# thangvubk/PESR

Measured on AMD Instinct MI355X. Metric: HR-patches/sec (x4 SR GAN train step, 48->192), higher is better.
Workload: dtype f32; 1 GPU; full GAN phase (G + D + VGG + RSGAN focal loss), per-GPU batch 16, LR 48x48 -> HR 192x192, 256 ch x 32 blocks; Adam lr 5e-07 instead of the reference's 5e-5 (same work per step; keeps D's loss O(0.1) on white-noise crops, see `lr_note`); global_batch=16, parallelism=dp1

## Files before the change

pesr_amd/csrc/conv3x3_mfma.hip:

```cpp
#include <mutex>
#include "common.h"
#include "launchers.h"
#include "conv_epilogue.h"

__device__ __attribute__((aligned(16))) const float g_zero16[4] = {0.f, 0.f, 0.f, 0.f};

__device__ __forceinline__ void lds_dma16(const float* gsrc, char* lds_wave_base) {
    __builtin_amdgcn_global_load_lds((const __attribute__((address_space(1))) void*)gsrc,
                                     (__attribute__((address_space(3))) void*)lds_wave_base, 16, 0, 0);
}

struct ConvArgs {
    const float* x;
    const float* wp;
    const float* bias;
    const float* skip;
    const float* mask;
    float* y;
    int N, H, W, Cin, Cout, OH, OW;
    int GH, GW;
    int TH, TW, tiles_x, tiles_y, n_tiles;
    int in_oy, in_ox;
    int HT, WT;
    int out_my, out_ay, out_mx, out_ax;
    int ntaps;
    unsigned long long tap_lo;
    unsigned tap_hi;
    float alpha, slope;
    int act;
    int ps;
    int cin_real;
    int cout_store;
    int ksplit;
    int chunks_per_split;
    float* slab;
    size_t slab_bytes;
    int ps_in;
    int bn_row0;
    int bn_mode, bn_cap;
    int dry;
    long bn_rows;
};

__device__ __forceinline__ unsigned tap_code(const ConvArgs& a, int t) {
    return t < 8 ? (unsigned)(a.tap_lo >> (8 * t)) & 0xffu : a.tap_hi;
}

template <int WAVES_M, int WAVES_N, int WM, int WN, int S, int HL, int MODE>
__device__ __forceinline__ void conv3x3_mfma_body(const ConvArgs& a, const int block_id, const int grid_blocks, const unsigned bn_kernarg_off) {
    constexpr int NT = WAVES_M * WAVES_N * 64;
    constexpr int BN = WAVES_N * WN * 16;
    constexpr int WL = (BN * 4 + NT - 1) / NT;
    extern __shared__ __attribute__((aligned(16))) char smem[];

    const int halo_pix = a.HT * a.WT;
    const int halo_bytes = ((halo_pix * 64 + 255) / 256) * 256;
    char* const halo0 = smem;
    char* const halo1 = smem + halo_bytes;
    char* const wb0 = smem + 2 * halo_bytes;

    const int tid = threadIdx.x, lane = tid & 63, wave = tid >> 6;
    const int wave_m = wave / WAVES_N, wave_n = wave % WAVES_N;
    const int r = lane & 15, g = lane >> 4;

    int lb = block_id;
    if ((grid_blocks & 7) == 0) lb = (lb & 7) * (grid_blocks >> 3) + (lb >> 3);
    const int tiles_total = a.n_tiles * a.tiles_x * a.tiles_y * a.N;
    const int ks = lb / tiles_total;
    int bid = lb - ks * tiles_total;
    const int nt = bid % a.n_tiles;  bid /= a.n_tiles;
    const int tx = bid % a.tiles_x;  bid /= a.tiles_x;
    const int ty = bid % a.tiles_y;
    const int img = bid / a.tiles_y;
    const int gy0 = ty * a.TH, gx0 = tx * a.TW;
    const int n0 = nt * BN;
    const int C16T = a.Cin >> 4;
    const int CB = ks * a.chunks_per_split;
    const int C16 = (C16T - CB) < a.chunks_per_split ? (C16T - CB) : a.chunks_per_split;

    int a_off[WM], b_off[WN];
#pragma unroll
    for (int i = 0; i < WM; ++i) {
        const int m = (wave_m * WM + i) * 16 + r;
        const int py = m / a.TW, px = m - py * a.TW;
        a_off[i] = ((py * S) * a.WT + (S == 2 ? px : px * S)) * 64 + g * 16;
    }
    const int WE = (a.WT + 1) >> 1;
#pragma unroll
    for (int j = 0; j < WN; ++j) b_off[j] = ((wave_n * WN + j) * 16 + r) * 64 + g * 16;

    const float* const xi = a.x + (size_t)img * a.H * a.W * a.cin_real;
    int h_src[HL];
#pragma unroll
    for (int k = 0; k < HL; ++k) {
        const int e = tid + k * NT;
        const int hp = e >> 2, q = e & 3;
        int off = -2;
        if (hp < halo_pix) {
            const int hy = hp / a.WT, sc = hp - hy * a.WT;
            const int hx = S == 2 ? (sc < WE ? 2 * sc : 2 * (sc - WE) + 1) : sc;
            const int iy = gy0 * S + a.in_oy + hy, ix = gx0 * S + a.in_ox + hx;
            if (iy >= 0 && iy < a.H && ix >= 0 && ix < a.W)
                off = a.ps_in ? ((2 * iy) * (2 * a.W) + 2 * ix) * (a.Cin >> 2) + q * 4 : (iy * a.W + ix) * a.cin_real + q * 4;
            else
                off = -1;
        }
        h_src[k] = off;
    }
    const float* const wn = a.wp + (size_t)n0 * 16;
    const size_t slab_stride = (size_t)a.Cout * 16;

    f32x4 acc[WM][WN];
#pragma unroll
    for (int i = 0; i < WM; ++i)
#pragma unroll
        for (int j = 0; j < WN; ++j) acc[i][j] = (f32x4){0.f, 0.f, 0.f, 0.f};

    f32x4 hreg[HL], wreg[WL];

    auto load_halo = [&](int c) {
        int coff = (CB + c) * 16;
        if (a.ps_in) coff = pesr_ps_in_chunk_off(coff, a.Cin >> 2, a.W);
        if (a.cin_real == 3) {
#pragma unroll
            for (int k = 0; k < HL; ++k) {
                const bool ok = h_src[k] >= 0 && ((tid + k * NT) & 3) == 0;
                const int o = ok ? h_src[k] : 0;
                const float v0 = xi[o], v1 = xi[o + 1], v2 = xi[o + 2];
                hreg[k] = ok ? (f32x4){v0, v1, v2, 0.f} : (f32x4){0.f, 0.f, 0.f, 0.f};
            }
            return;
        }
#pragma unroll
        for (int k = 0; k < HL; ++k) {
            const int o = h_src[k] < 0 ? 0 : h_src[k];
            f32x4 v = *(const f32x4*)(xi + o + coff);
            hreg[k] = h_src[k] >= 0 ? v : (f32x4){0.f, 0.f, 0.f, 0.f};
        }
    };
    auto store_halo = [&](char* hb) {
#pragma unroll
        for (int k = 0; k < HL; ++k)
            if (h_src[k] != -2) *(f32x4*)(hb + (tid + k * NT) * 16) = hreg[k];
    };
    auto load_w = [&](int c, int tw) {
        const float* src = wn + ((size_t)tw * C16T + CB + c) * slab_stride;
#pragma unroll
        for (int k = 0; k < WL; ++k) {
            const int e = tid + k * NT;
            if (BN * 4 % NT == 0 || e < BN * 4) wreg[k] = *(const f32x4*)(src + e * 4);
        }
    };
    auto store_w = [&](char* wb) {
#pragma unroll
        for (int k = 0; k < WL; ++k) {
            const int e = tid + k * NT;
            if (BN * 4 % NT == 0 || e < BN * 4) *(f32x4*)(wb + e * 16) = wreg[k];
        }
    };

    auto dma_w = [&](int c, int tw, char* wb) {
        const float* src = wn + ((size_t)tw * C16T + CB + c) * slab_stride;
#pragma unroll
        for (int k = 0; k < WL; ++k) {
            const int e = tid + k * NT;
            if (BN * 4 % NT == 0 || e < BN * 4) lds_dma16(src + e * 4, wb + (k * NT + wave * 64) * 16);
        }
    };
    auto dma_halo = [&](int c, char* hb) {
        int coff = (CB + c) * 16;
        if (a.ps_in) coff = pesr_ps_in_chunk_off(coff, a.Cin >> 2, a.W);
#pragma unroll
        for (int k = 0; k < HL; ++k) {
            if (h_src[k] != -2) {
                const float* src = h_src[k] >= 0 ? xi + h_src[k] + coff : g_zero16;
                lds_dma16(src, hb + (k * NT + wave * 64) * 16);
            }
        }
    };

    f32x4 fa0[WM], fb0[WN], fa1[WM], fb1[WN];

#define PESR_READ_FRAGS(FA, FB, C_, T_, WB_)                                                    \
    {                                                                                          \
        const char* const hb_ = ((C_) & 1) ? halo1 : halo0;                                    \
        const unsigned tc_ = tap_code(a, T_);                                                  \
        const int dx_ = (int)((tc_ >> 2) & 3u);                                                \
        const int toff_ = ((int)(tc_ & 3u) * a.WT + (S == 2 ? (dx_ == 1 ? WE : dx_ >> 1) : dx_)) * 64; \
        _Pragma("unroll") for (int i = 0; i < WM; ++i) FA[i] = *(const f32x4*)(hb_ + a_off[i] + toff_); \
        _Pragma("unroll") for (int j = 0; j < WN; ++j) FB[j] = *(const f32x4*)((WB_) + b_off[j]); \
    }
#define PESR_MFMA_BLOCK(FA, FB)                                                                 \
    _Pragma("unroll") for (int kk = 0; kk < 4; ++kk)                                            \
        _Pragma("unroll") for (int i = 0; i < WM; ++i)                                          \
            _Pragma("unroll") for (int j = 0; j < WN; ++j)                                      \
                acc[i][j] = __builtin_amdgcn_mfma_f32_16x16x4f32(FA[i][kk], FB[j][kk], acc[i][j], 0, 0, 0);

    const int nslab = C16 * a.ntaps;
    auto adv = [&](int& c_, int& t_) { if (++t_ == a.ntaps) { t_ = 0; if (++c_ == C16) c_ = 0; } };

    if (MODE == 2) {
        char* const ring = wb0;
        int cd = 0, td = 0, sd = 0;
        auto dma_next = [&]() { dma_w(cd, tap_code(a, td) >> 4, ring + (sd & 3) * (BN * 64)); adv(cd, td); ++sd; };
        dma_halo(0, halo0);
        dma_next(); dma_next(); dma_next();
        __syncthreads();
        int cr = 0, tr = 0, sr = 0;
        PESR_READ_FRAGS(fa0, fb0, cr, tr, ring + (sr & 3) * (BN * 64))  adv(cr, tr); ++sr;
        __syncthreads();
        int c = 0, t = 0;
#pragma unroll 1
        for (int sl = 0; sl < nslab; sl += 2) {
            dma_next(); dma_next();
            {
                int c1 = c, t1 = t; adv(c1, t1);
                const int copen = (t == 0) ? c : ((t1 == 0 && sl + 1 < nslab) ? c1 : -1);
                if (copen >= 0 && copen + 1 < C16 && (t == 0 || c1 != 0)) dma_halo(copen + 1, ((copen + 1) & 1) ? halo1 : halo0);
            }
            PESR_READ_FRAGS(fa1, fb1, cr, tr, ring + (sr & 3) * (BN * 64))  adv(cr, tr); ++sr;
            PESR_MFMA_BLOCK(fa0, fb0)
            adv(c, t);
            if (sl + 1 < nslab) {
                PESR_READ_FRAGS(fa0, fb0, cr, tr, ring + (sr & 3) * (BN * 64))  adv(cr, tr); ++sr;
                PESR_MFMA_BLOCK(fa1, fb1)
                adv(c, t);
            }
            __syncthreads();
        }
    } else {
        auto wslot = [&](int s_) -> char* { return wb0 + (MODE == 0 ? s_ % 3 : (s_ & 1)) * (BN * 64); };
        load_halo(0);
        load_w(0, tap_code(a, 0) >> 4);
        store_halo(halo0);
        store_w(wslot(0));
        if (nslab > 1) {
            int c1 = 0, t1 = 0; adv(c1, t1);
            load_w(c1, tap_code(a, t1) >> 4);
            store_w(wslot(1));
        }
        __syncthreads();
        if (MODE == 1) PESR_READ_FRAGS(fa0, fb0, 0, 0, wslot(0))
        int c = 0, t = 0;
#define PESR_STEP(CA, CB_, NA, NB, SL)                                                          \
        {                                                                                      \
            int c1 = c, t1 = t; adv(c1, t1);                                                   \
            int c2 = c1, t2 = t1; adv(c2, t2);                                                 \
            const bool halo_now = (t == 0) && (c + 1 < C16);                                   \
            load_w(c2, tap_code(a, t2) >> 4);                                                  \
            if (halo_now) load_halo(c + 1);                                                    \
            if (MODE == 1) PESR_READ_FRAGS(NA, NB, c1, t1, wslot((SL) + 1))                    \
            else PESR_READ_FRAGS(CA, CB_, c, t, wslot(SL))                                     \
            PESR_MFMA_BLOCK(CA, CB_)                                                           \
                        \
            __builtin_amdgcn_sched_barrier(0);                                                 \
            store_w(wslot((SL) + 2));        \
            if (halo_now) store_halo((c & 1) ? halo0 : halo1);                                 \
            __syncthreads();                                                                   \
            c = c1; t = t1;                                                                    \
        }
#pragma unroll 1
        for (int sl = 0; sl < nslab; sl += 2) {
            PESR_STEP(fa0, fb0, fa1, fb1, sl)
            if (sl + 1 < nslab) PESR_STEP(fa1, fb1, fa0, fb0, sl + 1)
        }
#undef PESR_STEP
    }
#undef PESR_MFMA_BLOCK
#undef PESR_READ_FRAGS

    const size_t img_out = (size_t)img * a.OH * a.OW;
    if (a.cout_store % 4 == 0) {
        constexpr int MT = WAVES_M * WM * 16;
        constexpr int C4 = BN / 4;
        constexpr int RS = BN * 4 + 16;
        constexpr int EIT = (MT * C4 + NT - 1) / NT;
        char* const ob = smem;
        const BnEpi* const bn = pesr_bn_epi(bn_kernarg_off);
        const int bn_mode = a.ksplit == 1 ? bn->mode : 0;
        const bool bn_on = bn_mode != 0;
        const float bn_slope = bn->slope;
        f32x4 st1 = {0.f, 0.f, 0.f, 0.f}, st2 = {0.f, 0.f, 0.f, 0.f};
        PesrBnCoef4 bnk = pesr_bn_coef4_zero();
        auto out_index = [&](int u, size_t* idx) -> bool {
            const int m = u / C4, c4 = u - m * C4;
            const int co = n0 + c4 * 4;
            const int py = m / a.TW, px = m - py * a.TW;
            const int gy = gy0 + py, gx = gx0 + px;
            if (u >= MT * C4 || gy >= a.GH || gx >= a.GW || co >= a.cout_store) return false;
            const int oy = gy * a.out_my + a.out_ay, ox = gx * a.out_mx + a.out_ax;
            if (a.ps) {
                *idx = pesr_ps_out_index(img, oy, ox, co, a.OH, a.OW, a.Cout);
            } else {
                *idx = (img_out + (size_t)oy * a.OW + ox) * a.cout_store + co;
            }
            return true;
        };
        f32x4 zpre[EIT];
        if (bn_mode == 2) {
            const int cq = n0 + (tid % C4) * 4;
            if (cq < a.cout_store) bnk = pesr_bn_coef4_load(bn, a.cout_store, cq);
        }
#pragma unroll
        for (int i = 0; i < WM; ++i)
#pragma unroll
            for (int jj = 0; jj < 4; ++jj) {
                const int m = (wave_m * WM + i) * 16 + g * 4 + jj;
#pragma unroll
                for (int j = 0; j < WN; ++j)
                    *(float*)(ob + m * RS + ((wave_n * WN + j) * 16 + r) * 4) = acc[i][j][jj];
            }
        __syncthreads();
        const size_t slab_off = (size_t)ks * ((size_t)a.N * a.OH * a.OW * a.cout_store);
        if (bn_mode == 2) {
            {
                const float* const bn_z = bn->z;
#pragma unroll
                for (int k = 0; k < EIT; ++k) {
                    size_t idx;
                    zpre[k] = out_index(tid + k * NT, &idx) ? *(const f32x4*)(bn_z + idx) : (f32x4){0.f, 0.f, 0.f, 0.f};
                }
            }
#pragma unroll
            for (int k = 0; k < EIT; ++k) {
                const int u = tid + k * NT;
                size_t idx;
                if (!out_index(u, &idx)) continue;
                const int m = u / C4, c4 = u - m * C4;
                const f32x4 v = pesr_bn_lrelu_grad4(*(const f32x4*)(ob + m * RS + c4 * 16) * a.alpha, zpre[k], bnk, bn_slope, st1, st2);
                *(f32x4*)(a.y + idx) = v;
            }
        } else {
            for (int u = tid; u < MT * C4; u += NT) {
                size_t idx;
                if (!out_index(u, &idx)) continue;
                const int m = u / C4, c4 = u - m * C4;
                const int co = n0 + c4 * 4;
                f32x4 v = *(const f32x4*)(ob + m * RS + c4 * 16);
                if (a.ksplit > 1) {
                    *(f32x4*)(a.slab + slab_off + idx) = v;
                    continue;
                }
                v = pesr_epi4_at(v, a.bias, co, a.alpha, a.mask, a.skip, idx, a.act, a.slope);
                if (bn_on) { st1 += v; st2 += v * v; }
                *(f32x4*)(a.y + idx) = v;
            }
        }
        if (bn_on) {
            __syncthreads();
            f32x4* const red = (f32x4*)smem;
            red[tid] = st1; red[NT + tid] = st2;
            __syncthreads();
            if (tid < C4 && n0 + tid * 4 < a.cout_store) {
                f64x4 d1 = {0.0, 0.0, 0.0, 0.0}, d2 = {0.0, 0.0, 0.0, 0.0};
                for (int k = 0; k < NT / C4; ++k) {
                    d1 += __builtin_convertvector(red[k * C4 + tid], f64x4);
                    d2 += __builtin_convertvector(red[NT + k * C4 + tid], f64x4);
                }
                const int row = a.bn_row0 + (img * a.tiles_y + ty) * a.tiles_x + tx;
                float* const pr = bn->part + (size_t)row * 2 * a.cout_store + n0 + tid * 4;
                *(f32x4*)pr = __builtin_convertvector(d1, f32x4);
                *(f32x4*)(pr + a.cout_store) = __builtin_convertvector(d2, f32x4);
            }
        }
        return;
    }
    float bias_r[WN];
#pragma unroll
    for (int j = 0; j < WN; ++j) {
        const int co = n0 + (wave_n * WN + j) * 16 + r;
        bias_r[j] = (a.bias && co < a.cout_store) ? a.bias[co] : 0.f;
    }
#pragma unroll
    for (int i = 0; i < WM; ++i) {
#pragma unroll
        for (int jj = 0; jj < 4; ++jj) {
            const int m = (wave_m * WM + i) * 16 + g * 4 + jj;
            const int py = m / a.TW, px = m - py * a.TW;
            const int gy = gy0 + py, gx = gx0 + px;
            if (gy >= a.GH || gx >= a.GW) continue;
            const int oy = gy * a.out_my + a.out_ay, ox = gx * a.out_mx + a.out_ax;
#pragma unroll
            for (int j = 0; j < WN; ++j) {
                const int co = n0 + (wave_n * WN + j) * 16 + r;
                if (co >= a.cout_store) continue;
                size_t idx;
                if (a.ksplit > 1) {
                    idx = (img_out + (size_t)oy * a.OW + ox) * a.cout_store + co;
                    a.slab[(size_t)ks * ((size_t)a.N * a.OH * a.OW * a.cout_store) + idx] = acc[i][j][jj];
                    continue;
                }
                if (a.ps) idx = pesr_ps_out_index(img, oy, ox, co, a.OH, a.OW, a.Cout);
                else idx = (img_out + (size_t)oy * a.OW + ox) * a.cout_store + co;
                a.y[idx] = pesr_epi1_at(acc[i][j][jj] + bias_r[j], nullptr, 0, a.alpha, a.mask, a.skip, idx, a.act, a.slope);
            }
        }
    }
}

template <int WAVES_M, int WAVES_N, int WM, int WN, int S, int HL, int MODE>
__global__ __launch_bounds__(WAVES_M* WAVES_N * 64) void conv3x3_mfma_kernel(const ConvArgs a, const BnEpi bn) {
    (void)bn;
    conv3x3_mfma_body<WAVES_M, WAVES_N, WM, WN, S, HL, MODE>(a, blockIdx.x, gridDim.x, (unsigned)((sizeof(ConvArgs) + 7) & ~(size_t)7));
}

struct ConvArgs4 {
    ConvArgs c[4];
    int tiles[4];
};
template <int WAVES_M, int WAVES_N, int WM, int WN, int HL>
__global__ __launch_bounds__(WAVES_M* WAVES_N * 64) void conv3x3_s2dgrad4_kernel(const ConvArgs4 a4, const BnEpi bn) {
    (void)bn;
    constexpr unsigned BO = (unsigned)((sizeof(ConvArgs4) + 7) & ~(size_t)7);
    const int bx = blockIdx.x;
    switch (blockIdx.y) {
        case 0: if (bx < a4.tiles[0]) conv3x3_mfma_body<WAVES_M, WAVES_N, WM, WN, 1, HL, 2>(a4.c[0], bx, a4.tiles[0], BO); break;
        case 1: if (bx < a4.tiles[1]) conv3x3_mfma_body<WAVES_M, WAVES_N, WM, WN, 1, HL, 1>(a4.c[1], bx, a4.tiles[1], BO); break;
        case 2: if (bx < a4.tiles[2]) conv3x3_mfma_body<WAVES_M, WAVES_N, WM, WN, 1, HL, 1>(a4.c[2], bx, a4.tiles[2], BO); break;
        default: if (bx < a4.tiles[3]) conv3x3_mfma_body<WAVES_M, WAVES_N, WM, WN, 1, HL, 0>(a4.c[3], bx, a4.tiles[3], BO); break;
    }
}

__global__ void conv_splitk_finish_kernel(const float* __restrict__ slab, const float* __restrict__ bias, const float* __restrict__ skip,
                                          const float* __restrict__ mask, float* __restrict__ y, long total, int C, int ksplit,
                                          float alpha, int act, float slope) {
    for (long e = (long)blockIdx.x * blockDim.x + threadIdx.x; e < total; e += (long)gridDim.x * blockDim.x) {
        float v = slab[e];
        for (int k = 1; k < ksplit; ++k) v += slab[(size_t)k * total + e];
        y[e] = pesr_epi1_at(v, bias, bias ? e % C : 0, alpha, mask, skip, e, act, slope);
    }
}
__global__ void conv_splitk_finish4_kernel(const f32x4* __restrict__ slab, const float* __restrict__ bias, const f32x4* __restrict__ skip,
                                           const f32x4* __restrict__ mask, f32x4* __restrict__ y, long total4, int C, int ksplit,
                                           float alpha, int act, float slope) {
    for (long e = (long)blockIdx.x * blockDim.x + threadIdx.x; e < total4; e += (long)gridDim.x * blockDim.x) {
        f32x4 p[8];
#pragma unroll
        for (int k = 0; k < 8; ++k)
            if (k < ksplit) p[k] = slab[(size_t)k * total4 + e];
        f32x4 v = p[0];
#pragma unroll
        for (int k = 1; k < 8; ++k)
            if (k < ksplit) v += p[k];
        y[e] = pesr_epi4_at(v, bias, (e * 4) % C, alpha, (const float*)mask, (const float*)skip, e * 4, act, slope);
    }
}

constexpr int PESR_BN_FINISH_ROWS = 256;
template <int MODE>
__global__ __launch_bounds__(256) void conv_splitk_finish4_bn_kernel(const f32x4* __restrict__ slab, const float* __restrict__ bias, f32x4* __restrict__ y,
                                                                      long total4, int C, int ksplit, float alpha, const BnEpi bn) {
    const int C4 = C >> 2;
    const int c4 = (int)(((long)blockIdx.x * 256 + threadIdx.x) % C4);
    f32x4 st1 = {0.f, 0.f, 0.f, 0.f}, st2 = st1, b4 = st1;
    PesrBnCoef4 bnk = pesr_bn_coef4_zero();
    if (MODE == 2) bnk = pesr_bn_coef4_load(&bn, C, c4 * 4);
    if (bias) b4 = *(const f32x4*)(bias + c4 * 4);
    for (long e = (long)blockIdx.x * 256 + threadIdx.x; e < total4; e += (long)gridDim.x * 256) {
        f32x4 p[8];
#pragma unroll
        for (int k = 0; k < 8; ++k)
            if (k < ksplit) p[k] = slab[(size_t)k * total4 + e];
        f32x4 v = p[0];
#pragma unroll
        for (int k = 1; k < 8; ++k)
            if (k < ksplit) v += p[k];
        v = (v + b4) * alpha;
        if (MODE == 2) {
            v = pesr_bn_lrelu_grad4(v, ((const f32x4*)bn.z)[e], bnk, bn.slope, st1, st2);
        } else {
            st1 += v; st2 += v * v;
        }
        y[e] = v;
    }
    __shared__ f32x4 red[2][256];
    red[0][threadIdx.x] = st1; red[1][threadIdx.x] = st2;
    __syncthreads();
    const int cw = C4 < 256 ? C4 : 256;
    if (threadIdx.x < cw) {
        f64x4 d1 = {0.0, 0.0, 0.0, 0.0}, d2 = {0.0, 0.0, 0.0, 0.0};
        for (int k = threadIdx.x; k < 256; k += cw) {
            d1 += __builtin_convertvector(red[0][k], f64x4);
            d2 += __builtin_convertvector(red[1][k], f64x4);
        }
        float* const pr = bn.part + (size_t)blockIdx.x * 2 * C + c4 * 4;
        *(f32x4*)pr = __builtin_convertvector(d1, f32x4);
        *(f32x4*)(pr + C) = __builtin_convertvector(d2, f32x4);
    }
}

long pesr_conv_splitk_finish_bn_rows(int C, int ksplit) {
    const int C4 = C >> 2;
    if (C % 4 || ksplit > 8 || C4 < 1 || (C4 < 256 ? 256 % C4 : C4 % 256)) return 0;
    return PESR_BN_FINISH_ROWS;
}

int pesr_conv_splitk_finish_bn_launch(const float* slab, const float* bias, float* y, long total, int C, int ksplit, float alpha, const BnEpi& bn,
                                      hipStream_t stream) {
    if (!pesr_conv_splitk_finish_bn_rows(C, ksplit) || !bn.part) return PESR_EINVAL;
    const long total4 = total / 4;
    if (bn.mode == 2)
        hipLaunchKernelGGL(conv_splitk_finish4_bn_kernel<2>, dim3(PESR_BN_FINISH_ROWS), dim3(256), 0, stream, (const f32x4*)slab, bias, (f32x4*)y, total4, C, ksplit,
                           alpha, bn);
    else
        hipLaunchKernelGGL(conv_splitk_finish4_bn_kernel<1>, dim3(PESR_BN_FINISH_ROWS), dim3(256), 0, stream, (const f32x4*)slab, bias, (f32x4*)y, total4, C, ksplit,
                           alpha, bn);
    return pesr_launch_status();
}

int pesr_conv_splitk_finish_launch(const float* slab, const float* bias, const float* skip, const float* mask, float* y, long total,
                                   int C, int ksplit, float alpha, int act, float slope, hipStream_t stream) {
    if (C % 4 == 0 && ksplit <= 8) {
        const long total4 = total / 4;
        const int fgrid = (int)((total4 + 255) / 256 < 4096 ? (total4 + 255) / 256 : 4096);
        hipLaunchKernelGGL(conv_splitk_finish4_kernel, dim3(fgrid), dim3(256), 0, stream, (const f32x4*)slab, bias, (const f32x4*)skip,
                           (const f32x4*)mask, (f32x4*)y, total4, C, ksplit, alpha, act, slope);
        return pesr_launch_status();
    }
    const int fgrid = (int)((total + 255) / 256 < 2048 ? (total + 255) / 256 : 2048);
    hipLaunchKernelGGL(conv_splitk_finish_kernel, dim3(fgrid), dim3(256), 0, stream, slab, bias, skip, mask, y, total, C, ksplit, alpha,
                       act, slope);
    return pesr_launch_status();
}

namespace {

static thread_local BnEpi g_bn_epi;

static void set_tap(ConvArgs& a, int t, int dy, int dx, int w) {
    const unsigned long long code = (unsigned)(dy | (dx << 2) | (w << 4));
    if (t < 8) a.tap_lo |= code << (8 * t); else a.tap_hi = (unsigned)code;
}

struct TileChoice { int TH, TW; };

static bool choose_tile(int MT, int S, int hext, int wext, int GH, int GW, int max_halo_pix, TileChoice* out) {
    long best = -1;
    for (int TW = 1; TW <= MT; ++TW) {
        if (MT % TW) continue;
        const int TH = MT / TW;
        const int HTl = (TH - 1) * S + hext, WTl = (TW - 1) * S + wext;
        if ((long)HTl * WTl > max_halo_pix) continue;
        const long cover = (long)pesr_cdiv(GH, TH) * TH * pesr_cdiv(GW, TW) * TW;
        const long score = cover * 4096 + (long)HTl * WTl;
        if (best < 0 || score < best) { best = score; out->TH = TH; out->TW = TW; }
    }
    return best >= 0;
}

template <int WAVES_M, int WAVES_N, int WM, int WN, int S, int HL>
static int prep_cfg(ConvArgs& a, int hext, int wext, int target_wgs, size_t* lds_out, int* mode_out, long* grid_out) {
    constexpr int NT = WAVES_M * WAVES_N * 64;
    constexpr int MT = WAVES_M * WM * 16;
    constexpr int BN = WAVES_N * WN * 16;
    if (a.Cout % BN) return PESR_EINVAL;
    TileChoice tc;
    const int max_halo = (HL * NT) / 4;
    if (!choose_tile(MT, S, hext, wext, a.GH, a.GW, max_halo, &tc)) return PESR_EINVAL;
    a.TH = tc.TH; a.TW = tc.TW;
    a.HT = (a.TH - 1) * S + hext; a.WT = (a.TW - 1) * S + wext;
    a.tiles_y = pesr_cdiv(a.GH, a.TH); a.tiles_x = pesr_cdiv(a.GW, a.TW);
    a.n_tiles = a.Cout / BN;
    const int halo_bytes = ((a.HT * a.WT * 64 + 255) / 256) * 256;
    const int mode = (a.ntaps >= 4 && a.cin_real != 3) ? 2 : (a.ntaps > 1 ? 1 : 0);
    size_t lds = 2 * (size_t)halo_bytes + (mode == 2 ? 4 : (mode == 0 ? 3 : 2)) * (size_t)BN * 64;
    const size_t lds_acc = (size_t)MT * (BN * 4 + 16);
    if (lds_acc > lds) lds = lds_acc;
    if (lds > 160 * 1024) return PESR_EINVAL;
    const long tiles = (long)a.N * a.tiles_y * a.tiles_x * a.n_tiles;
    const int C16T = a.Cin / 16;
    a.ksplit = 1; a.chunks_per_split = C16T;
    const size_t out_bytes = (size_t)a.N * a.OH * a.OW * a.cout_store * sizeof(float);
    if (a.slab && tiles < (long)target_wgs * 5 / 8 && a.out_my == 1 && a.out_mx == 1 && !a.ps && C16T >= 8) {
        int want = (int)((target_wgs + tiles - 1) / tiles);
        if (want > 8) want = 8;
        if (want > C16T / 4) want = C16T / 4;
        while (want > 1 && (size_t)want * out_bytes > a.slab_bytes) --want;
        if (want > 1) {
            a.chunks_per_split = (C16T + want - 1) / want;
            a.ksplit = (C16T + a.chunks_per_split - 1) / a.chunks_per_split;
        }
    }
    *lds_out = lds; *mode_out = mode; *grid_out = tiles * a.ksplit;
    return PESR_OK;
}

template <int WAVES_M, int WAVES_N, int WM, int WN, int S, int HL>
static int launch_cfg(ConvArgs& a, int hext, int wext, hipStream_t stream, int target_wgs = 256) {
    constexpr int NT = WAVES_M * WAVES_N * 64;
    size_t lds; int mode; long grid;
    const int rc = prep_cfg<WAVES_M, WAVES_N, WM, WN, S, HL>(a, hext, wext, target_wgs, &lds, &mode, &grid);
    if (rc) return rc;
    a.bn_rows = (a.cout_store % 4 == 0 && NT % (WAVES_N * WN * 4) == 0 && !a.ps)
                    ? (a.ksplit == 1 ? (long)a.N * a.tiles_y * a.tiles_x : pesr_conv_splitk_finish_bn_rows(a.cout_store, a.ksplit)) : 0;
    if (a.dry) return PESR_OK;
    if (a.bn_mode && (a.bn_rows == 0 || a.bn_row0 + a.bn_rows != a.bn_cap || !g_bn_epi.part)) return PESR_EINVAL;
    const size_t out_bytes = (size_t)a.N * a.OH * a.OW * a.cout_store * sizeof(float);
    const float* bias = a.bias; const float* skip = a.skip; const float* mask = a.mask;
    BnEpi a_bn = g_bn_epi;
    if (a.ksplit > 1) a_bn.mode = 0;
#define PESR_LAUNCH_MODE(M_)                                                                              \
    {                                                                                                      \
        auto kern = conv3x3_mfma_kernel<WAVES_M, WAVES_N, WM, WN, S, HL, M_>;                              \
        static PesrDeviceOnce attr_once;                                        \
        attr_once([&] {                                                           \
            (void)hipFuncSetAttribute((const void*)kern, hipFuncAttributeMaxDynamicSharedMemorySize, 160 * 1024); \
        });                                                                                                  \
        hipLaunchKernelGGL(kern, dim3((unsigned)grid), dim3(NT), lds, stream, a, a_bn);                    \
    }
    if (mode == 2) PESR_LAUNCH_MODE(2) else if (mode == 1) PESR_LAUNCH_MODE(1) else PESR_LAUNCH_MODE(0)
#undef PESR_LAUNCH_MODE
    if (a.ksplit > 1 && g_bn_epi.mode) {
        if (skip || mask || a.act != PESR_ACT_NONE) return PESR_EINVAL;
        return pesr_conv_splitk_finish_bn_launch((const float*)a.slab, bias, a.y, (long)(out_bytes / sizeof(float)), a.cout_store, a.ksplit, a.alpha,
                                                 g_bn_epi, stream);
    }
    if (a.ksplit > 1)
        return pesr_conv_splitk_finish_launch((const float*)a.slab, bias, skip, mask, a.y, (long)(out_bytes / sizeof(float)), a.cout_store,
                                              a.ksplit, a.alpha, a.act, a.slope, stream);
    return pesr_launch_status();
}

template <int WAVES_M, int WAVES_N, int WM, int WN, int HL>
static int launch_s2dgrad4(ConvArgs4& a4, const int* hext, const int* wext, hipStream_t stream) {
    constexpr int NT = WAVES_M * WAVES_N * 64;
    size_t lds = 0; long gmax = 0;
    long rows = 0;
    const bool rows_ok = a4.c[0].cout_store % 4 == 0 && NT % (WAVES_N * WN * 4) == 0;
    for (int k = 0; k < 4; ++k) {
        a4.tiles[k] = 0;
        a4.c[k].bn_row0 = (int)rows;
        if (a4.c[k].GH <= 0 || a4.c[k].GW <= 0) continue;
        size_t l; int mode; long grid;
        const int rc = prep_cfg<WAVES_M, WAVES_N, WM, WN, 1, HL>(a4.c[k], hext[k], wext[k], 256, &l, &mode, &grid);
        if (rc) return rc;
        if (mode != (k == 0 ? 2 : (k == 3 ? 0 : 1)) || a4.c[k].ksplit != 1) return PESR_EINVAL;
        a4.tiles[k] = (int)grid;
        rows += (long)a4.c[k].N * a4.c[k].tiles_y * a4.c[k].tiles_x;
        if (l > lds) lds = l;
        if (grid > gmax) gmax = grid;
    }
    a4.c[0].bn_rows = rows_ok ? rows : 0;
    if (a4.c[0].dry) return PESR_OK;
    if (a4.c[0].bn_mode && (!rows_ok || rows != a4.c[0].bn_cap || !g_bn_epi.part)) return PESR_EINVAL;
    if (gmax == 0) return PESR_OK;
    auto kern = conv3x3_s2dgrad4_kernel<WAVES_M, WAVES_N, WM, WN, HL>;
    static PesrDeviceOnce attr_once;
    attr_once([&] { (void)hipFuncSetAttribute((const void*)kern, hipFuncAttributeMaxDynamicSharedMemorySize, 160 * 1024); });
    hipLaunchKernelGGL(kern, dim3((unsigned)gmax, 4), dim3(NT), lds, stream, a4, g_bn_epi);
    return pesr_launch_status();
}

template <int S>
static int dispatch(ConvArgs& a, int hext, int wext, hipStream_t stream) {
    const long M = (long)a.N * a.GH * a.GW;
    if (S == 2 && a.ntaps == 9 && a.Cout == 64 && M >= 64 * 512) return launch_cfg<1, 4, 4, 1, S, 5>(a, hext, wext, stream);
    if (a.Cout % 64 == 0 && a.Cout >= 128 && (long)pesr_cdiv(M, 144) * (a.Cout / 64) <= 320)
        return launch_cfg<1, 4, 3, 1, S, (S == 1 ? 2 : 4)>(a, hext, wext, stream, 768);
    if (a.Cout % 256 == 0) {
        const long tiles_big = (M / 144) * (a.Cout / 256);
        if (tiles_big >= 192) return launch_cfg<1, 8, 9, 2, S, (S == 1 ? 2 : 6)>(a, hext, wext, stream);
    }
    if (a.Cout % 128 == 0) {
        const long tiles = (M / 144) * (a.Cout / 128);
        if (tiles >= 192) return launch_cfg<1, 8, 9, 1, S, (S == 1 ? 2 : 6)>(a, hext, wext, stream);
    }
    if (a.Cout % 64 == 0) return launch_cfg<1, 4, 9, 1, S, (S == 1 ? 4 : 11)>(a, hext, wext, stream);
    if (a.Cout == 16 && S == 1) return launch_cfg<4, 1, 4, 1, 1, 6>(a, hext, wext, stream);
    return PESR_EINVAL;
}

}

static void set_bn(ConvArgs& a, PesrBnFuseArgs* f) {
    a.bn_mode = 0; a.dry = 0; a.bn_rows = 0; a.bn_row0 = 0; a.bn_cap = 0;
    g_bn_epi = BnEpi{};
    if (!f) return;
    a.dry = f->dry;
    if (f->dry || !f->mode) return;
    a.bn_mode = f->mode; a.bn_cap = f->rows;
    g_bn_epi.mode = f->mode; g_bn_epi.slope = f->slope; g_bn_epi.part = f->part;
    g_bn_epi.z = f->z; g_bn_epi.mi = f->mean_invstd; g_bn_epi.gamma = f->gamma; g_bn_epi.beta = f->beta;
}

int pesr_conv3x3_launch(const float* x, const float* wp, const float* bias, const float* skip, const float* mask,
                        float* y, int N, int H, int W, int Cin, int Cout, int stride, float alpha, int act,
                        float slope, int ps, int ps_in, int flip, int cin_real, int cout_store, void* ws, size_t ws_bytes,
                        hipStream_t stream, PesrBnFuseArgs* fuse) {
    if (cin_real == 0) cin_real = Cin;
    if (cout_store == 0) cout_store = Cout;
    if ((cin_real != Cin && (cin_real != 3 || Cin != 16 || ps_in)) || (cout_store != Cout && ps)) return PESR_EINVAL;
    if (ps_in && (Cin % 64 || stride != 1)) return PESR_EINVAL;
    if (ps && Cout % 4) return PESR_EINVAL;
    if (Cin % 16 || (stride != 1 && stride != 2) || N <= 0 || H <= 0 || W <= 0) return PESR_EINVAL;
    ConvArgs a{};
    a.x = x; a.wp = wp; a.bias = bias; a.skip = skip; a.mask = mask; a.y = y;
    a.N = N; a.H = H; a.W = W; a.Cin = Cin; a.Cout = Cout;
    a.OH = (H - 1) / stride + 1; a.OW = (W - 1) / stride + 1;
    a.GH = a.OH; a.GW = a.OW;
    a.in_oy = -1; a.in_ox = -1;
    a.out_my = 1; a.out_ay = 0; a.out_mx = 1; a.out_ax = 0;
    a.ntaps = 9;
    for (int t = 0; t < 9; ++t) set_tap(a, t, t / 3, t % 3, flip ? 8 - t : t);
    a.alpha = alpha; a.slope = slope; a.act = act; a.ps = ps; a.ps_in = ps_in;
    a.cin_real = cin_real; a.cout_store = cout_store;
    a.slab = (float*)ws; a.slab_bytes = ws_bytes;
    set_bn(a, fuse);
    if (fuse && fuse->mode == 2 && (mask || skip || bias || act != PESR_ACT_NONE)) return PESR_EINVAL;
    const int rc = stride == 1 ? dispatch<1>(a, 3, 3, stream) : dispatch<2>(a, 3, 3, stream);
    if (fuse) fuse->rows_out = rc ? 0 : a.bn_rows;
    return rc;
}

int pesr_conv3x3_s2_dgrad_launch(const float* dy, const float* wp, const float* mask, float* dx, int N, int H, int W,
                                 int Cout_fwd, int Cin_fwd, float alpha, hipStream_t stream, PesrBnFuseArgs* fuse) {
    if (Cout_fwd % 16) return PESR_EINVAL;
    const int OH = (H - 1) / 2 + 1, OW = (W - 1) / 2 + 1;
    ConvArgs4 a4{};
    int hext[4], wext[4];
    for (int k = 0; k < 4; ++k) {
        const int py = k < 2 ? 1 : 0, px = (k == 0 || k == 2) ? 1 : 0;
        ConvArgs& a = a4.c[k];
        a.x = dy; a.wp = wp; a.bias = nullptr; a.skip = nullptr; a.mask = mask; a.y = dx;
        a.N = N; a.H = OH; a.W = OW; a.Cin = Cout_fwd; a.Cout = Cin_fwd;
        a.OH = H; a.OW = W;
        a.GH = (H - py + 1) / 2; a.GW = (W - px + 1) / 2;
        a.in_oy = 0; a.in_ox = 0;
        a.out_my = 2; a.out_ay = py; a.out_mx = 2; a.out_ax = px;
        int kys[2], dys[2], nky, kxs[2], dxs[2], nkx;
        if (py == 0) { nky = 1; kys[0] = 1; dys[0] = 0; } else { nky = 2; kys[0] = 0; dys[0] = 1; kys[1] = 2; dys[1] = 0; }
        if (px == 0) { nkx = 1; kxs[0] = 1; dxs[0] = 0; } else { nkx = 2; kxs[0] = 0; dxs[0] = 1; kxs[1] = 2; dxs[1] = 0; }
        a.ntaps = 0;
        for (int i = 0; i < nky; ++i)
            for (int j = 0; j < nkx; ++j) {
                set_tap(a, a.ntaps, dys[i], dxs[j], kys[i] * 3 + kxs[j]);
                ++a.ntaps;
            }
        a.alpha = alpha; a.slope = 0.f; a.act = PESR_ACT_NONE; a.ps = 0; a.ps_in = 0;
        a.cin_real = Cout_fwd; a.cout_store = Cin_fwd;
        a.slab = nullptr; a.slab_bytes = 0; a.ksplit = 1;
        set_bn(a, fuse);
        hext[k] = py + 1; wext[k] = px + 1;
    }
    if (fuse && fuse->mode == 2 && mask) return PESR_EINVAL;
    if (fuse) fuse->rows_out = 0;
    const int Cout = Cin_fwd;
    const long M = (long)N * a4.c[0].GH * a4.c[0].GW;
    if (Cout % 64) {
        if (fuse && !fuse->dry && fuse->mode) return PESR_EINVAL;
        if (fuse && fuse->dry) return PESR_OK;
        for (int k = 0; k < 4; ++k) {
            if (a4.c[k].GH <= 0 || a4.c[k].GW <= 0) continue;
            const int rc = dispatch<1>(a4.c[k], hext[k], wext[k], stream);
            if (rc) return rc;
        }
        return PESR_OK;
    }
    int rc;
    if (Cout >= 128 && (long)pesr_cdiv(M, 144) * (Cout / 64) <= 320) rc = launch_s2dgrad4<1, 4, 3, 1, 2>(a4, hext, wext, stream);
    else if (Cout % 256 == 0 && 4 * (M / 144) * (Cout / 256) >= 192) rc = launch_s2dgrad4<1, 8, 9, 2, 2>(a4, hext, wext, stream);
    else if (Cout % 128 == 0 && 4 * (M / 144) * (Cout / 128) >= 192) rc = launch_s2dgrad4<1, 8, 9, 1, 2>(a4, hext, wext, stream);
    else rc = launch_s2dgrad4<1, 4, 9, 1, 4>(a4, hext, wext, stream);
    if (fuse) fuse->rows_out = rc ? 0 : a4.c[0].bn_rows;
    return rc;
}
```

Measured before the change: 304.0 patches/s.

## Add MODE 3 conv path streaming weights from global into registers

Adds a new conv3x3 MFMA kernel mode for single-wave-row, stride-2, 9-tap configurations. Weights are loaded straight from global memory into registers three taps ahead, instead of being DMA'd into an LDS ring, which frees LDS and removes barriers for weight staging. The halo is still double-buffered in LDS through register fetch-and-land, with one barrier per channel chunk. This trades LDS traffic and synchronisation for more VGPR pressure and exposed global-load latency. It is on by default and can be turned off with an environment variable.

```diff
diff --git a/pesr_amd/csrc/conv3x3_mfma.hip b/pesr_amd/csrc/conv3x3_mfma.hip
--- a/pesr_amd/csrc/conv3x3_mfma.hip
+++ b/pesr_amd/csrc/conv3x3_mfma.hip
@@ -199,7 +199,99 @@
     const int nslab = C16 * a.ntaps;
     auto adv = [&](int& c_, int& t_) { if (++t_ == a.ntaps) { t_ = 0; if (++c_ == C16) c_ = 0; } };
 
-    if (MODE == 2) {
+    if (MODE == 3) {
+        static_assert(MODE != 3 || WAVES_M == 1, "MODE 3: the weights are not shared between waves");
+        constexpr int NT3 = 9;
+        const float* wl[WN];
+#pragma unroll
+        for (int j = 0; j < WN; ++j) wl[j] = wn + (b_off[j] >> 2);
+        f32x4 fa[2][WM], fb[3][WN];
+        auto fetch_halo = [&](int c_) {
+            int coff = (CB + c_) * 16;
+            if (a.ps_in) coff = pesr_ps_in_chunk_off(coff, a.Cin >> 2, a.W);
+#pragma unroll
+            for (int k = 0; k < HL; ++k) hreg[k] = *(const f32x4*)(xi + (h_src[k] < 0 ? 0 : h_src[k]) + coff);
+        };
+        auto land_halo = [&](char* hb) {
+#pragma unroll
+            for (int k = 0; k < HL; ++k)
+                if (h_src[k] != -2) *(f32x4*)(hb + (tid + k * NT) * 16) = h_src[k] >= 0 ? hreg[k] : (f32x4){0.f, 0.f, 0.f, 0.f};
+        };
+        auto load_b = [&](f32x4* FB, int c_, int t_) {
+#ifndef PESR_M3_NO_WLOAD
+            const size_t so = ((size_t)(tap_code(a, t_) >> 4) * C16T + CB + c_) * slab_stride;
+#pragma unroll
+            for (int j = 0; j < WN; ++j) FB[j] = *(const f32x4*)(wl[j] + so);
+#endif
+        };
+        auto read_a = [&](f32x4* FA, int c_, int t_) {
+            const char* const hb = (c_ & 1) ? halo1 : halo0;
+            const unsigned tc = tap_code(a, t_);
+            const int dx = (int)((tc >> 2) & 3u);
+            const int toff = ((int)(tc & 3u) * a.WT + (S == 2 ? (dx == 1 ? WE : dx >> 1) : dx)) * 64;
+#pragma unroll
+            for (int i = 0; i < WM; ++i) FA[i] = *(const f32x4*)(hb + a_off[i] + toff);
+        };
+#if defined(PESR_M3_NO_HALO)
+#define PESR_M3_HALO_FETCH(C_)
+#define PESR_M3_HALO_LAND(C_)
+#define PESR_M3_WAIT() asm volatile("s_waitcnt lgkmcnt(0)" ::: "memory");
+#elif defined(PESR_M3_DMA_HALO)
+#define PESR_M3_HALO_FETCH(C_) dma_halo(C_, ((C_) & 1) ? halo1 : halo0);
+#define PESR_M3_HALO_LAND(C_)
+#define PESR_M3_WAIT() asm volatile("s_waitcnt vmcnt(%0) lgkmcnt(0)" ::"n"(3 * WN) : "memory");
+#else
+#define PESR_M3_HALO_FETCH(C_) fetch_halo(C_);
+#define PESR_M3_HALO_LAND(C_) land_halo(((C_) & 1) ? halo1 : halo0);
+#define PESR_M3_WAIT() asm volatile("s_waitcnt lgkmcnt(0)" ::: "memory");
+#endif
+#ifdef PESR_M3_NO_BARRIER
+#define PESR_M3_BARRIER()
+#else
+#define PESR_M3_BARRIER() PESR_M3_WAIT() __builtin_amdgcn_s_barrier();
+#endif
+        fetch_halo(0);
+        load_b(fb[0], 0, 0);
+        load_b(fb[1], 0, 1);
+        land_halo(halo0);
+        __syncthreads();
+        read_a(fa[0], 0, 0);
+        int c = 0;
+#define PESR_STEP3(U_)                                                                          \
+        {                                                                                      \
+            constexpr int u = (U_), t = u % NT3;                                               \
+             \
+            {                                                                                  \
+                int c2 = c + (t + 2 >= NT3 ? 1 : 0);                                           \
+                if (t + 2 >= NT3 && c2 == C16) c2 = 0;                                         \
+                load_b(fb[(u + 2) % 3], c2, (t + 2) % NT3);                                    \
+            }                                                                                  \
+            if (t == 0 && c + 1 < C16) { PESR_M3_HALO_FETCH(c + 1) }                           \
+             \
+            __builtin_amdgcn_sched_barrier(0);                                                 \
+            if (t == NT3 - 1) {                                                                \
+                if (c + 1 < C16) { PESR_M3_HALO_LAND(c + 1) }                                  \
+                PESR_M3_BARRIER()                                                              \
+                __builtin_amdgcn_sched_barrier(0);                                             \
+            }                                                                                  \
+            if (!(t == NT3 - 1 && c + 1 == C16)) read_a(fa[(u + 1) & 1], t == NT3 - 1 ? c + 1 : c, (t + 1) % NT3);   \
+             \
+            __builtin_amdgcn_sched_barrier(0);                                                 \
+            PESR_MFMA_BLOCK(fa[u & 1], fb[u % 3])                                              \
+            if (t == NT3 - 1 && ++c == C16) break;                                             \
+        }
+#pragma unroll 1
+        for (;;) {
+            PESR_STEP3(0) PESR_STEP3(1) PESR_STEP3(2) PESR_STEP3(3) PESR_STEP3(4) PESR_STEP3(5)
+            PESR_STEP3(6) PESR_STEP3(7) PESR_STEP3(8) PESR_STEP3(9) PESR_STEP3(10) PESR_STEP3(11)
+            PESR_STEP3(12) PESR_STEP3(13) PESR_STEP3(14) PESR_STEP3(15) PESR_STEP3(16) PESR_STEP3(17)
+        }
+#undef PESR_STEP3
+#undef PESR_M3_BARRIER
+#undef PESR_M3_WAIT
+#undef PESR_M3_HALO_LAND
+#undef PESR_M3_HALO_FETCH
+    } else if (MODE == 2) {
         char* const ring = wb0;
         int cd = 0, td = 0, sd = 0;
         auto dma_next = [&]() { dma_w(cd, tap_code(a, td) >> 4, ring + (sd & 3) * (BN * 64)); adv(cd, td); ++sd; };
@@ -548,6 +640,16 @@
     return best >= 0;
 }
 
+static bool stream_w_enabled() {
+    const char* const e = getenv("PESR_MFMA_STREAMW");
+    return !(e && e[0] == '0' && !e[1]);
+}
+
+template <int WAVES_M, int WAVES_N, int WM, int WN, int S>
+constexpr bool stream_w_cfg(int ntaps) {
+    return WAVES_M == 1 && S == 2 && ntaps == 9 && ((WAVES_N == 4 && (WM == 3 || WM == 4)) || (WAVES_N == 8 && WM == 9 && WN == 1));
+}
+
 template <int WAVES_M, int WAVES_N, int WM, int WN, int S, int HL>
 static int prep_cfg(ConvArgs& a, int hext, int wext, int target_wgs, size_t* lds_out, int* mode_out, long* grid_out) {
     constexpr int NT = WAVES_M * WAVES_N * 64;
@@ -562,8 +664,9 @@
     a.tiles_y = pesr_cdiv(a.GH, a.TH); a.tiles_x = pesr_cdiv(a.GW, a.TW);
     a.n_tiles = a.Cout / BN;
     const int halo_bytes = ((a.HT * a.WT * 64 + 255) / 256) * 256;
-    const int mode = (a.ntaps >= 4 && a.cin_real != 3) ? 2 : (a.ntaps > 1 ? 1 : 0);
-    size_t lds = 2 * (size_t)halo_bytes + (mode == 2 ? 4 : (mode == 0 ? 3 : 2)) * (size_t)BN * 64;
+    int mode = (a.ntaps >= 4 && a.cin_real != 3) ? 2 : (a.ntaps > 1 ? 1 : 0);
+    if (mode == 2 && stream_w_cfg<WAVES_M, WAVES_N, WM, WN, S>(a.ntaps) && stream_w_enabled()) mode = 3;
+    size_t lds = 2 * (size_t)halo_bytes + (mode == 3 ? 0 : (mode == 2 ? 4 : (mode == 0 ? 3 : 2))) * (size_t)BN * 64;
     const size_t lds_acc = (size_t)MT * (BN * 4 + 16);
     if (lds_acc > lds) lds = lds_acc;
     if (lds > 160 * 1024) return PESR_EINVAL;
@@ -608,7 +711,9 @@
         });                                                                                                  \
         hipLaunchKernelGGL(kern, dim3((unsigned)grid), dim3(NT), lds, stream, a, a_bn);                    \
     }
-    if (mode == 2) PESR_LAUNCH_MODE(2) else if (mode == 1) PESR_LAUNCH_MODE(1) else PESR_LAUNCH_MODE(0)
+    if (mode == 3) {
+        if constexpr (stream_w_cfg<WAVES_M, WAVES_N, WM, WN, S>(9)) PESR_LAUNCH_MODE(3) else return PESR_EINVAL;
+    } else if (mode == 2) PESR_LAUNCH_MODE(2) else if (mode == 1) PESR_LAUNCH_MODE(1) else PESR_LAUNCH_MODE(0)
 #undef PESR_LAUNCH_MODE
     if (a.ksplit > 1 && g_bn_epi.mode) {
         if (skip || mask || a.act != PESR_ACT_NONE) return PESR_EINVAL;
```

Measured after the change: 304.7 patches/s (median of 6 runs). No clear change (+0.2%).
